# m7a/bo-lz4-ada

Measured on AMD Instinct MI355X. Metric: decompressed MiB/s + achieved HBM GB/s vs roofline, 4MiB-block frame @1/2/4/8 GPU, higher is better.
Workload: dtype u8; 1 GPU; configs[2] size, configs[3] shape: 2048 x 4 MiB independent blocks = 8 GiB decoded, FLG 0x70 (B.Indep|B.Checksum), BD 0x70 (content-checksum variant FLG 0x74: e2e_content_checksum); class=mixed, blocks_total=2048, blocks_per_gpu=2048, block_max=4194304, compressed_bytes_rank0=4214903424, decoded_bytes_rank0=8589934592, parallelism=block-shard x1

## Files before the change

### bo-lz4-ada_amd/csrc/lz4ada_idx.hip

```cpp
#include <hip/hip_runtime.h>
#include <stdint.h>

#include "lz4ada_internal.h"
#include "lz4ada_dev.h"

namespace lz4ada {
namespace idx {

#ifndef LZ4ADA_STORED_NT
#define LZ4ADA_STORED_NT 2
#endif
constexpr int CHUNK = 16384;
constexpr int SUB = 32;
constexpr int BATCH = 64 * SUB;
constexpr int RING = 4 * BATCH;
constexpr int LONG = 256;
constexpr int32_t MAX_RUN = 1 << 28;
#ifndef LZ4ADA_LEAD_SEQ
#define LZ4ADA_LEAD_SEQ 60
#endif
constexpr int32_t LEAD_SEQ = LZ4ADA_LEAD_SEQ;
#ifndef LZ4ADA_LEAD_MAX
#define LZ4ADA_LEAD_MAX 1024
#endif
// ... 844 lines not shown
		has = next_item(S, cp, co, cpart, sub_end, n, o_batch, it);
	if (__any(has)) {
		vm_wait();
		for (;;) {
			const uint64_t m = __ballot(has);
			if (m == 0)
				break;
			const int32_t leader = __builtin_ctzll(m);
			const int32_t ldst = __shfl(it.dst, leader);
			const int32_t llen = __shfl(it.len, leader);
			const int32_t lsrc = __shfl(it.src, leader);
			bool ready;
			if (llen > LONG) {
				if (lsrc >= 0)
					wave_literal(ob, ldst, S, lsrc, llen);
				else
					wave_match(ob, olim, ldst, -lsrc, llen);
				ready = (lane == leader);
			} else {
				ready = has && it.len <= LONG &&
				        (it.src >= 0 || it.dst + it.src + min(-it.src, it.len) <= ldst);
				if (ready) {
					if (it.src >= 0)
						for (int32_t c = 0; c < it.len; c += 16)
							gstore_n(ob + it.dst + c, fetch16(S, it.src + c), min(16, it.len - c));
					else
						lane_match(ob, olim, it.dst, -it.src, it.len);
				}
			}
			vm_wait();
			if (ready)
				has = next_item(S, cp, co, cpart, sub_end, n, o_batch, it);
		}
	}
	return true;
}

constexpr int OW = 4080;
constexpr int ORING = 8192;
constexpr int OMASK = ORING - 1;
constexpr int MAXSEQ = 128;
constexpr int RMAX = MAXSEQ / 64;
constexpr int GC = 1;
constexpr int FLUSH_ST = (OW + 15) / 16 / 64 + 1;
static_assert(2 * OW + 16 <= ORING, "batch + its HBM threshold must fit the ring");
#ifndef LZ4ADA_OW_CUT
#define LZ4ADA_OW_CUT OW
#endif
#ifndef LZ4ADA_SEQ_CUT
#define LZ4ADA_SEQ_CUT MAXSEQ
#endif

struct alignas(16) DecLds {
	uint8_t ring[RING + 16];
	uint8_t oring[ORING];
	uint16_t cst[MAXSEQ];
	uint8_t own[256];
	uint64_t rrec[4 * 64];
	uint64_t ldesc[2 * 64];
	uint32_t plut[16 * 4];
	uint8_t junk[16];
};
static_assert(sizeof(DecLds) <= 20480, "8 waves per CU: at most 20 KiB of LDS per wave");

__device__ __forceinline__ uint8_t* oring_of(DecLds& D) { return D.oring; }
__device__ __forceinline__ const uint8_t* oring_of(const DecLds& D) { return D.oring; }
__device__ __forceinline__ uint8_t* own_of(DecLds& D) { return D.own; }
__device__ __forceinline__ uint64_t* ldesc_of(DecLds& D) { return D.ldesc; }
template <class LD>
struct lds_fast {
	static constexpr bool value = false;
};
template <>
struct lds_fast<DecLds> {
	static constexpr bool value = true;
};
__device__ __forceinline__ uint8_t* junk_of(DecLds& D) { return D.junk; }
__device__ __forceinline__ const uint32_t* plut_of(const DecLds& D) { return D.plut; }
template <class LD>
__device__ __forceinline__ uint8_t* junk_of(LD&) { return nullptr; }
template <class LD>
__device__ __forceinline__ const uint32_t* plut_of(const LD&) { return nullptr; }
template <class LD>
__device__ __forceinline__ constexpr uint32_t omask_of(const LD&) { return OMASK; }

__device__ __forceinline__ void lds_store_bf(uint8_t* p, uint8_t* junk, u32x4 v, uint32_t n)
{
	const uint64_t lo = uint64_t(v.x) | (uint64_t(v.y) << 32);
	const uint64_t hi = uint64_t(v.z) | (uint64_t(v.w) << 32);
	__builtin_memcpy(n >= 16u ? p : junk, &v, 16);
	__builtin_memcpy((n & 8u) ? p : junk, &lo, 8);
	const uint64_t r8 = (n & 8u) ? hi : lo;
	uint8_t* const p4 = p + (n & 8u);
	const uint32_t w4 = uint32_t(r8);
	__builtin_memcpy((n & 4u) ? p4 : junk, &w4, 4);
	const uint32_t r4 = (n & 4u) ? uint32_t(r8 >> 32) : w4;
	uint8_t* const p2 = p4 + (n & 4u);
	const uint16_t w2 = uint16_t(r4);
	__builtin_memcpy((n & 2u) ? p2 : junk, &w2, 2);
	*((n & 1u) ? p2 + (n & 2u) : junk) = uint8_t((n & 2u) ? (r4 >> 16) : r4);
}

template <class LD>
__device__ __forceinline__ void ostore(LD& L, int32_t x, u32x4 v, int32_t n)
{
	const uint32_t a = uint32_t(x) & omask_of(L);
	if constexpr (lds_fast<LD>::value) {
		if (__builtin_expect(!__any(a + uint32_t(n) > omask_of(L) + 1), 1)) {
			lds_store_bf(&oring_of(L)[a], junk_of(L), v, uint32_t(n));
			return;
		}
	}
	if (a + uint32_t(n) <= omask_of(L) + 1) {
		lds_store_n(&oring_of(L)[a], v, n);
		return;
	}
	const uint64_t lo = uint64_t(v.x) | (uint64_t(v.y) << 32);
	const uint64_t hi = uint64_t(v.z) | (uint64_t(v.w) << 32);
	for (int32_t i = 0; i < n; ++i) {
		const uint64_t w = i < 8 ? lo : hi;
		oring_of(L)[(a + uint32_t(i)) & omask_of(L)] = uint8_t(w >> (8 * (i & 7)));
	}
}

template <class LD>
__device__ __forceinline__ u32x4 oload16(const LD& L, int32_t x)
{
	return ring16(oring_of(L), uint32_t(x) & omask_of(L), omask_of(L));
}

constexpr uint64_t pattern_lut()
{
	uint64_t v = 0;
	for (int o = 1; o <= 8; ++o)
		v |= (uint64_t(o * (16 / o)) << (5 * (o - 1))) | (uint64_t(8 % o) << (40 + 2 * (o - 1)));
	return v;
}
constexpr uint64_t PAT_LUT = pattern_lut();

__device__ __forceinline__ void make_pattern16(uint64_t s0, uint64_t s1, int32_t off, u32x4& pv,
                                               int32_t& stp)
{
	uint64_t x, hi;
	if (off <= 8) {
		x = off == 8 ? s0 : (s0 & ((uint64_t(1) << (8 * off)) - 1));
#pragma unroll
		for (int i = 0; i < 3; ++i) {
			const int32_t w = off << i;
			x |= w < 8 ? x << (8 * w) : 0;
		}
		const uint32_t sh = uint32_t(off - 1);
		stp = int32_t((PAT_LUT >> (5 * sh)) & 31u);
		const int32_t r = int32_t((PAT_LUT >> (40 + 2 * sh)) & 3u);
		hi = r == 0 ? x : (x >> (8 * r)) | ((x >> (8 * (8 - off))) << (8 * (8 - r)));
	} else {
		const int32_t r = off - 8;
		x = s0;
		hi = (s1 & ((uint64_t(1) << (8 * r)) - 1)) | (s0 << (8 * r));
		stp = off;
	}
	pv.x = uint32_t(x);
	pv.y = uint32_t(x >> 32);
	pv.z = uint32_t(hi);
	pv.w = uint32_t(hi >> 32);
}

__device__ __forceinline__ u32x4 merge_at(u32x4 a, u32x4 b, int32_t c)
{
	auto m = [c](int32_t d) -> uint32_t {
		const int32_t t = c - 4 * d;
		return t >= 4 ? ~0u : (t <= 0 ? 0u : (1u << (8 * t)) - 1u);
	};
	u32x4 v;
	v.x = (a.x & m(0)) | (b.x & ~m(0));
	v.y = (a.y & m(1)) | (b.y & ~m(1));
	v.z = (a.z & m(2)) | (b.z & ~m(2));
	v.w = (a.w & m(3)) | (b.w & ~m(3));
	return v;
}

__device__ __forceinline__ int32_t pattern_step(int32_t off)
{
	return off <= 8 ? int32_t((PAT_LUT >> (5 * (off - 1))) & 31u) : off;
}

__device__ __forceinline__ void pattern_lut_init(uint32_t* plut)
{
	const uint32_t l = lane_id(), off = l >> 2, d = l & 3u;
	uint32_t sel = 0;
	if (off > 0)
		for (uint32_t t = 0; t < 4; ++t) {
			const uint32_t idx = (4 * d + t) % off;
			uint32_t x = idx;
			if (off > 8 && d == 2 && idx >= 8)
				x = idx - 4;
			if (off >= 12 && d == 3 && idx >= 12)
				x = idx - 8;
			sel |= x << (8 * t);
		}
	plut[l] = sel;
}

__device__ __forceinline__ u32x4 pattern_perm(u32x4 v, int32_t off, const uint32_t* plut)
{
	const u32x4 sel = *reinterpret_cast<const u32x4*>(plut + 4 * off);
	const uint32_t h2 = off <= 8 ? v.y : v.z, h3 = off <= 11 ? v.y : v.w;
	u32x4 o;
	o.x = __builtin_amdgcn_perm(v.y, v.x, sel.x);
	o.y = __builtin_amdgcn_perm(v.y, v.x, sel.y);
	o.z = __builtin_amdgcn_perm(h2, v.x, sel.z);
	o.w = __builtin_amdgcn_perm(h3, v.x, sel.w);
	return o;
}

template <class LD>
__device__ __forceinline__ void ring_match(LD& L, int32_t dst, int32_t off, int32_t len)
{
	const int32_t src = dst - off;
	u32x4 pv = oload16(L, src);
	int32_t stp = 16;
	const bool pat = off < 16 && off < len;
	if (pat) {
		if constexpr (lds_fast<LD>::value) {
			pv = pattern_perm(pv, off, plut_of(L));
			stp = pattern_step(off);
		} else {
			make_pattern16(uint64_t(pv.x) | (uint64_t(pv.y) << 32), uint64_t(pv.z) | (uint64_t(pv.w) << 32),
			               off, pv, stp);
		}
	}
	ostore(L, dst, pv, min(16, len));
	int32_t start = 0;
	for (int32_t x = stp; x < len; x += stp) {
		u32x4 v = pv;
		if (!pat) {
			start += 16;
			if (start >= off)
				start -= off;
			v = oload16(L, src + start);
			if (off - start < 16)
				v = merge_at(v, oload16(L, src + start - off), off - start);
		}
		ostore(L, dst + x, v, min(16, len - x));
	}
}

__device__ __forceinline__ int32_t div_small(int32_t t, int32_t d, int32_t& r)
{
	int32_t q = int32_t(float(t) * __builtin_amdgcn_rcpf(float(d)));
	r = t - q * d;
	if (r < 0) {
		--q;
		r += d;
	}
	if (r >= d) {
		++q;
		r -= d;
	}
	return q;
}


__device__ __forceinline__ int32_t piece_owner(int32_t inc, int32_t t);

template <class LD>
__device__ __forceinline__ int32_t chunk_owner(LD& D, int32_t inc, int32_t np, int32_t t0)
{
	const int32_t lane = int32_t(lane_id());
	const int32_t seed = __popcll(__ballot(inc <= t0));
	uint8_t* own = own_of(D);
	own[lane] = uint8_t(lane == 0 ? seed : 0);
	const int32_t excl = inc - np;
	if (np > 0 && excl >= t0 && excl < t0 + 64)
		own[excl - t0] = uint8_t(lane);
	wave_lds_fence();
	const int32_t v = own[lane];
	wave_lds_fence();
	return wave_incl_max(v);
}

template <class LD>
__device__ __forceinline__ int32_t chunk_owner2(LD& D, int32_t inc0, int32_t np0, int32_t inc1,
                                                int32_t np1, int32_t t0)
{
	const int32_t lane = int32_t(lane_id());
	const int32_t seed = __popcll(__ballot(inc0 <= t0)) + __popcll(__ballot(inc1 <= t0));
	uint8_t* own = own_of(D);
	own[lane] = uint8_t(lane == 0 ? seed : 0);
	const int32_t e0 = inc0 - np0, e1 = inc1 - np1;
	if (np0 > 0 && e0 >= t0 && e0 < t0 + 64)
		own[e0 - t0] = uint8_t(lane);
	if (np1 > 0 && e1 >= t0 && e1 < t0 + 64)
		own[e1 - t0] = uint8_t(64 + lane);
	wave_lds_fence();
	const int32_t v = own[lane];
	wave_lds_fence();
	return wave_incl_max(v);
}

__device__ __forceinline__ int32_t match_pieces(int32_t off, int32_t ml)
{
	if (ml <= 0)
		return 0;
	if (!(off < 16 && off < ml))
		return (ml + 15) >> 4;
	const int32_t stp = pattern_step(off);
	int32_t rr;
	return stp == 16 ? (ml + 15) >> 4 : div_small(ml + stp - 1, stp, rr);
}

#ifndef LZ4ADA_BORROW_SLOTS
#define LZ4ADA_BORROW_SLOTS 2
#endif
constexpr int BORROW_SLOTS = LZ4ADA_BORROW_SLOTS;
static_assert(BORROW_SLOTS >= 0 && BORROW_SLOTS <= 2, "round 0's slots, or both rounds'");

#ifndef LZ4ADA_FWD_ROUNDS
#define LZ4ADA_FWD_ROUNDS 5
#endif
constexpr int FWD_ROUNDS = LZ4ADA_FWD_ROUNDS;
#ifndef LZ4ADA_FWD_PIECES
#define LZ4ADA_FWD_PIECES 0
#endif
constexpr int FWD_PIECES = LZ4ADA_FWD_PIECES;

template <class LD>
__device__ __forceinline__ int32_t ring_pieces(LD& D, const int32_t (&mdst)[RMAX],
                                               const int32_t (&off)[RMAX], const int32_t (&ml)[RMAX],
                                               int32_t o_batch, int32_t glo = INT32_MIN)
{
	int32_t steps = 0;
	const int32_t lane = int32_t(lane_id());
	const int32_t np0 = match_pieces(off[0], ml[0]), np1 = match_pieces(off[1], ml[1]);
	const int32_t inc0 = wave_incl_scan(np0);
	const int32_t tot0 = __shfl(inc0, 63);
	const int32_t inc1 = tot0 + wave_incl_scan(np1);
	const int32_t tot = __shfl(inc1, 63);
	auto pack = [&](int32_t md, int32_t of, int32_t m, int32_t excl) -> uint64_t {
		return uint64_t(uint16_t(md - o_batch)) | (uint64_t(uint16_t(of)) << 16) |
		       (uint64_t(uint16_t(m)) << 32) | (uint64_t(uint16_t(excl)) << 48);
	};
	uint64_t* ldesc = ldesc_of(D);
	ldesc[lane] = pack(mdst[0], off[0], ml[0], inc0 - np0);
	ldesc[64 + lane] = pack(mdst[1], off[1], ml[1], inc1 - np1);
	for (int32_t t0 = 0; t0 < tot; t0 += 64) {
		const int32_t t = t0 + lane;
		const bool act = t < tot;
		const int32_t lo = min(chunk_owner2(D, inc0, np0, inc1, np1, t0), 127);
		const uint64_t dd = ldesc[lo];
		const int32_t od = o_batch + int32_t(dd & 0xffffu);
		const int32_t ooff = int32_t((dd >> 16) & 0xffffu), oml = int32_t((dd >> 32) & 0xffffu);
		const int32_t k = t - int32_t(dd >> 48);
		const bool opat = ooff < 16 && ooff < oml;
		const int32_t ostp = opat ? pattern_step(ooff) : 16;
		const bool wide = !opat && oml > ooff;
		const int32_t pd = od + k * ostp;
		const int32_t pn = min(16, oml - k * ostp);
		const int32_t s_lo = (opat || wide) ? od - ooff : od - ooff + 16 * k;
		const int32_t s_hi = (opat || wide) ? od : s_lo + pn;
		const int32_t pe = act ? pd + pn : INT32_MAX, ps = act ? pd : INT32_MAX;
		int32_t fj1 = 64, fj2 = -1;
		if (!__all(!act || s_hi <= __shfl(ps, 0))) {
			int32_t j1 = 0, c2 = 0;
#pragma unroll
			for (int st = 32; st >= 1; st >>= 1) {
				if (__shfl(pe, j1 + st - 1) <= s_lo)
					j1 += st;
				if (__shfl(ps, c2 + st - 1) < s_hi)
					c2 += st;
			}
			fj1 = j1;
			fj2 = min(c2 - 1, lane - 1);
		}
		int32_t F = 0;
		if (FWD_PIECES > 0 && glo != INT32_MIN) {
			const bool plain = act && !opat && !wide;
			int32_t sh = ooff;
			const int32_t q0 = __shfl(ps, fj1), qe = __shfl(pe, fj1);
			bool fw = act && fj1 == fj2 && q0 <= s_lo && s_hi <= qe && __shfl(int32_t(plain), fj1) != 0;
			for (int r = 0; r < FWD_PIECES && __any(fw); ++r) {
				const int32_t p = fj1;
				const int32_t qs = __shfl(sh, p), q1 = __shfl(fj1, p), q2 = __shfl(fj2, p);
				const bool qf = __shfl(int32_t(fw), p) != 0;
				if (fw && s_lo - F - qs >= glo) {
					F += qs;
					sh = ooff + F;
					fj1 = q1;
					fj2 = q2;
					fw = qf;
				} else {
					fw = false;
				}
			}
		}
		uint64_t dep = 0;
		if (act && fj1 <= fj2)
			dep = (fj2 == 63 ? ~uint64_t(0) : ((uint64_t(2) << fj2) - 1)) & ~((uint64_t(1) << fj1) - 1);
		int32_t rem = 0;
		if (wide)
			div_small(16 * k, ooff, rem);
		const int32_t a1 = (opat ? od - ooff : (wide ? od - ooff + rem : s_lo)) - F;
		const int32_t cut = (wide && ooff - rem < 16) ? ooff - rem : 16;
		bool pend = act;
		for (;;) {
			const uint64_t pm = __ballot(pend);
			if (pm == 0)
				break;
			const bool ready = pend && (dep & pm) == 0;
			if constexpr (lds_fast<LD>::value) {
				u32x4 v = oload16(D, a1);
				if (ready && cut < 16)
					v = merge_at(v, oload16(D, a1 - ooff), cut);
				if (ready && opat)
					v = pattern_perm(v, ooff, plut_of(D));
				ostore(D, pd, v, ready ? pn : 0);
			} else if (ready) {
				u32x4 v = oload16(D, a1);
				if (cut < 16)
					v = merge_at(v, oload16(D, a1 - ooff), cut);
				if (opat) {
					int32_t sstp;
					make_pattern16(uint64_t(v.x) | (uint64_t(v.y) << 32),
					               uint64_t(v.z) | (uint64_t(v.w) << 32), ooff, v, sstp);
				}
				ostore(D, pd, v, pn);
			}
			pend = pend && !ready;
			wave_lds_fence();
			++steps;
		}
	}
	return steps;
}

#ifndef LZ4ADA_RING_LANE_MAX
#define LZ4ADA_RING_LANE_MAX 32
#endif
constexpr int RING_LANE_MAX = LZ4ADA_RING_LANE_MAX;
template <class LD>
__device__ __forceinline__ int32_t ring_lanes(LD& D, int32_t mdst, int32_t off, int32_t ml,
                                           int32_t rbeg, int32_t L, int32_t glo = INT32_MIN)
{
	const int32_t lane = int32_t(lane_id());
	const int32_t src = mdst - off;
	const int32_t dep_end = src + min(off, ml);
	const bool far = ml > 0 && (dep_end <= rbeg || off <= L);
	int32_t steps = 0;
	if (!__any(ml > 0 && !far)) {
		if (far)
			ring_match(D, mdst, off, ml);
		wave_lds_fence();
		return 0;
	}
	bool near = ml > 0;
	const int32_t mend = mdst + ml;
	int32_t j1 = 0, c2 = 0;
#pragma unroll
	for (int st = 32; st >= 1; st >>= 1) {
		if (__shfl(mend, j1 + st - 1) <= src)
			j1 += st;
		if (__shfl(mdst, c2 + st - 1) < dep_end)
			c2 += st;
	}
	int32_t fj1 = far ? 64 : j1, fj2 = far ? -1 : min(c2 - 1, lane - 1);
	int32_t fo = off;
	{
		const int32_t pm = __shfl(mdst, fj1), pe = __shfl(mend, fj1), po = __shfl(off, fj1);
		const bool pn = __shfl(int32_t(near), fj1) != 0;
		bool fw = FWD_ROUNDS > 0 && glo != INT32_MIN && near && off >= ml && fj1 == fj2 && pm <= src &&
		          dep_end <= pe && pn && po >= pe - pm;
		for (int r = 0; r < FWD_ROUNDS && __any(fw); ++r) {
			const int32_t p = fj1;
			const int32_t qo = __shfl(fo, p), q1 = __shfl(fj1, p), q2 = __shfl(fj2, p);
			const bool qf = __shfl(int32_t(fw), p) != 0;
			if (fw && mdst - fo - qo >= glo) {
				fo += qo;
				fj1 = q1;
				fj2 = q2;
				fw = qf;
			} else {
				fw = false;
			}
		}
	}
	uint64_t dep = 0;
	if (near && fj1 <= fj2)
		dep = (fj2 == 63 ? ~uint64_t(0) : ((uint64_t(2) << fj2) - 1)) & ~((uint64_t(1) << fj1) - 1);
	for (;;) {
		const uint64_t pending = __ballot(near);
		if (pending == 0)
			break;
		const bool ready = near && (dep & pending) == 0;
		if (ready) {
			ring_match(D, mdst, fo, ml);
			near = false;
		}
		wave_lds_fence();
		++steps;
	}
	return steps;
}

__device__ __forceinline__ int32_t piece_owner(int32_t inc, int32_t t)
{
	int32_t lo = 0;
#pragma unroll
	for (int st = 32; st >= 1; st >>= 1)
		if (__shfl(inc, lo + st - 1) <= t)
// ... 430 lines not shown
					const int32_t t = t0 + lane;
					const int32_t lo = min(chunk_owner2(D, inc0, nc0, inc1, nc1, t0), 127);
					const uint64_t dd = D.ldesc[lo];
					const int32_t lit = base + int32_t(dd & 0xffffu);
					const int32_t dst = o_batch + int32_t((dd >> 16) & 0xffffu);
					const int32_t L = int32_t((dd >> 32) & 0xffffu);
					const int32_t k = 1 + t - int32_t(dd >> 48);
					const bool has = t < tot;
					ostore(D, dst + 16 * k, ZL ? u32x4{ 0u, 0u, 0u, 0u } : fetch16(S, has ? lit + 16 * k : S.lo),
					       has ? min(16, L - 16 * k) : 0);
				}
			}
		}
		wave_lds_fence();
		ISTAMP(D_LIT);

		int32_t mring[RMAX], oring[RMAX], lring[RMAX];
		__builtin_amdgcn_s_waitcnt(0x0F70);
		ostore(D, rpd, vr, rpn);
#pragma unroll
		for (int r = 0; r < RMAX; ++r) {
			mring[r] = oring[r] = lring[r] = 0;
			if (64 * r < N) {
				const int32_t mdst = rdst[r] + rL[r], off = roff[r], ml = rml[r];
				const bool hbm = ml > 0 && mdst - off < glo;
				static_assert(GC == 1, "one own HBM piece per match");
				ostore(D, hbm ? mdst : o_batch + (bpc[r] & 0xfff), vg[r][0], hbm ? min(16, ml) : bpc[r] >> 12);
				int32_t xoff = off, xml = (ml > 0 && !hbm) ? ml : 0;
				if (d1p) {
					int32_t k1 = 0, sp = S.lo, gq = 0;
					bool fo = false;
					if (ml > 0 && n1 + mdst < off && oph - off < 8) {
						const int32_t dd = oph - off;
						const int32_t ovs = rL[r] > 0 ? 8 * ((rL[r] + 7) >> 3) - rL[r] : rlit[r] & 7;
						if (dd < ovs) {
							k1 = min(ovs - dd, ml);
							if (rL[r] > 0) {
								sp = rlit[r] + rL[r] + dd;
							} else {
								gq = (rlit[r] >> 3) - D1_QBIAS + dd;
								fo = true;
							}
						}
					}
					if (fo && gq >= glo) {
						xoff = mdst - gq;
						xml = k1;
						k1 = 0;
						fo = false;
					}
					u32x4 v = ZL ? u32x4{ 0u, 0u, 0u, 0u } : fetch16(S, sp);
					if (fo)
						__builtin_memcpy(&v, ob + gq, 16);
					ostore(D, mdst, v, k1);
				}
				if (rtot[r] > rfirst[r]) {
					ICOUNT(D_HSLOW_B, r == 0 || rtot[0] <= rfirst[0]);
					ICOUNT(D_HSLOW_P, rtot[r] - rfirst[r]);
					const int32_t nc = hbm ? max(((ml + 15) >> 4) - GC, 0) : 0;
					const int32_t inc = wave_incl_scan(nc);
					for (int32_t t0 = rfirst[r]; t0 < rtot[r]; t0 += 64) {
						const int32_t t = t0 + lane;
						const int32_t lo = piece_owner(inc, t);
						const int32_t k = GC + t - (__shfl(inc, lo) - __shfl(nc, lo));
						const int32_t osrc = __shfl(mdst - off, lo), odst = __shfl(mdst, lo);
						const int32_t oml = __shfl(ml, lo);
						if (t < rtot[r]) {
							u32x4 v;
							__builtin_memcpy(&v, ob + osrc + 16 * k, 16);
							ostore(D, odst + 16 * k, v, min(16, oml - 16 * k));
						}
					}
					__builtin_amdgcn_s_waitcnt(0x0F70);
				}
				mring[r] = mdst;
				oring[r] = xoff;
				lring[r] = xml;
			}
		}
		wave_lds_fence();
		ISTAMP(D_MFAR);
		static_assert(RMAX == 2, "ring dealing pairs two rounds");
		if (__any(lring[0] > RING_LANE_MAX || lring[1] > RING_LANE_MAX)) {
			const int32_t st = ring_pieces(D, mring, oring, lring, o_batch, glo);
			ICOUNT(D_TASKS, 1);
			ICOUNT(D_ROUNDS, st);
#ifdef LZ4ADA_IDX_STAMPS
			{
				const int32_t tot = __shfl(wave_incl_scan(match_pieces(oring[0], lring[0]) +
				                                          match_pieces(oring[1], lring[1])), 63);
				ICOUNT(D_RCHUNKS, (tot + 63) >> 6);
				ICOUNT(D_ROVF_B, tot > 64);
				ICOUNT(D_ROVF_P, max(tot - 64, 0));
			}
#endif
			(void)st;
		} else {
#pragma unroll
			for (int r = 0; r < RMAX; ++r) {
				if (64 * r < N) {
					const int32_t st = ring_lanes(D, mring[r], oring[r], lring[r], rbeg[r], rL[r], glo);
					ICOUNT(D_GBATCHES, 1);
					ICOUNT(D_LANES, st);
					(void)st;
				}
			}
		}
		ISTAMP(D_NEAR);

		{
			const int32_t u0 = o_batch >> 4, u1 = o_end >> 4;
#pragma unroll
			for (int i = 0; i < FLUSH_ST; ++i) {
				const int32_t u = u0 + lane + 64 * i;
				if (u < u1)
					*reinterpret_cast<GLOBAL u32x4*>(ob + (u << 4)) =
					    *reinterpret_cast<const u32x4*>(&D.oring[(u << 4) & OMASK]);
			}
		}
		o_batch = o_end;
		k0 += m;
		ISTAMP(D_FLUSH);
	}
	d1 = __any(d1);
	deep = __any(deep);
	if (ZL)
		hcnt = __shfl(wave_incl_scan(hcnt), 63);
	if (!bad && lane == 0 && (o_batch & 15))
		gstore_n(ob + (o_batch & ~15), *reinterpret_cast<const u32x4*>(&D.oring[(o_batch & ~15) & OMASK]),
		         o_batch & 15);
	if (lane == 0) {
		if (bad) {
			status[b].code = DS_RETRY;
		} else {
			status[b].code = DS_OK;
			status[b].aux = (d1 ? AUX_D1_RISK : 0) | (d1p ? AUX_D1_EMU : 0) | (deep ? AUX_DEEP_HIST : 0);
			status[b].detail = ZL ? hcnt : 0;
			status[b].err_out_pos = 0;
			status[b].out_len = uint32_t(o_batch);
		}
	}
	ISTAMP_FLUSH();
	out_len = bad ? 0 : o_batch;
	return bad ? DS_RETRY : DS_OK;
}

enum KIdxMode : int {
	K_PASS2 = 0,
	K_SERIAL = 1,
	K_HIST = 2,
	K_FUSED = 3,
};

__global__ __launch_bounds__(64) __attribute__((amdgpu_waves_per_eu(2))) void k_decode_idx(const uint8_t* __restrict__ frame,
                                                    uint64_t frame_len,
                                                    const lz4ada_block_desc* __restrict__ desc,
                                                    uint32_t nblocks, uint8_t* __restrict__ tab_all,
                                                    uint8_t* __restrict__ out,
                                                    lz4ada_block_status* __restrict__ status,
                                                    int mode)
{
	__shared__ union {
		DecLds d;
		IdxLds<1> x;
	} U;
	DecLds& D = U.d;
	if (mode == K_FUSED) {
		if (blockIdx.x < nblocks)
			index_block<1>(U.x, frame, frame_len, desc, blockIdx.x, tab_all, status);
		vm_wait();
		__builtin_amdgcn_fence(__ATOMIC_SEQ_CST, "workgroup");
		__syncthreads();
		mode = K_PASS2;
	}
	const bool serial = mode == K_SERIAL;
	int64_t hist = mode == K_HIST ? LINK_HIST : 0;
	uint32_t b = serial ? 0u : blockIdx.x;
	const uint32_t bend = serial ? nblocks : min(blockIdx.x + 1u, nblocks);
	for (; b < bend; ++b) {
		int32_t len;
		const int32_t code = decode_block(D, frame, frame_len, desc, b, tab_all, out, status,
		                                  hist, len);
		if (!serial)
			return;
		vm_wait();
		__syncthreads();
		if (code != DS_OK)
			break;
		if (b + 1 < nblocks && (uint32_t(len) != desc[b].out_cap ||
		                        desc[b + 1].out_off != desc[b].out_off + uint64_t(len))) {
			++b;
			break;
		}
		hist += len;
	}
	if (!serial)
		return;
	for (uint32_t r = b + lane_id(); r < nblocks; r += 64)
		if (status[r].code == DS_OK || r > b)
			status[r].code = DS_RETRY;
}


__global__ __launch_bounds__(64) __attribute__((amdgpu_waves_per_eu(2))) void k_decode_idx_zl(
        const uint8_t* __restrict__ frame, uint64_t frame_len, const lz4ada_block_desc* __restrict__ desc,
        uint32_t nblocks, uint8_t* __restrict__ tab_all, uint8_t* __restrict__ out,
        lz4ada_block_status* __restrict__ status)
{
	__shared__ DecLds D;
	if (blockIdx.x >= nblocks)
		return;
	int32_t len;
	decode_block(D, frame, frame_len, desc, blockIdx.x, tab_all, out, status, LINK_HIST, len, true, true);
}

__global__ __launch_bounds__(64) __attribute__((amdgpu_waves_per_eu(2))) void k_decode_idx_lk(
        const uint8_t* __restrict__ frame, uint64_t frame_len, const lz4ada_block_desc* __restrict__ desc,
        uint32_t nblocks, uint8_t* __restrict__ tab_all, uint8_t* __restrict__ out,
        lz4ada_block_status* __restrict__ status)
{
	__shared__ DecLds D;
	if (blockIdx.x >= nblocks)
		return;
	int32_t len;
	decode_block(D, frame, frame_len, desc, blockIdx.x, tab_all, out, status, LINK_HIST, len, false, true);
}


constexpr int ORING2 = 16384;
constexpr int32_t RFLOOR2 = ORING2 - 2 * OW;
static_assert(OW + 16 + 128 + 16 < RFLOOR2, "the HBM threshold must lie inside the kept window");

struct alignas(16) PpLds2 {
	uint8_t ring[RING + 16];
	uint8_t oring[ORING2];
	uint64_t rrec[4 * 64];
	uint64_t ldesc[2][2 * 64];
	uint16_t cst[2][MAXSEQ];
	uint8_t own[2][256];
	int32_t tok;
	int32_t staged;
	int32_t abort_;
	int32_t pad;
	int32_t done[2];
};

struct WP2 {
	PpLds2& L;
	int32_t w;
};
__device__ __forceinline__ uint8_t* oring_of(WP2& V) { return V.L.oring; }
__device__ __forceinline__ const uint8_t* oring_of(const WP2& V) { return V.L.oring; }
__device__ __forceinline__ uint8_t* own_of(WP2& V) { return V.L.own[V.w]; }
__device__ __forceinline__ uint64_t* ldesc_of(WP2& V) { return V.L.ldesc[V.w]; }
__device__ __forceinline__ constexpr uint32_t omask_of(const WP2&) { return ORING2 - 1; }

__device__ __forceinline__ int32_t lds_peek(const int32_t* p)
{
	return __builtin_amdgcn_readfirstlane(*reinterpret_cast<const volatile int32_t*>(p));
}

__device__ __forceinline__ void lds_publish(int32_t* p, int32_t v)
{
	asm volatile("" ::: "memory");
	__builtin_amdgcn_s_waitcnt(0xC07F);
	*reinterpret_cast<volatile int32_t*>(p) = v;
	asm volatile("" ::: "memory");
}

__device__ __forceinline__ bool lds_wait_ge(int32_t* abort_flag, const int32_t* p, int32_t want)
{
	for (uint32_t it = 0; lds_peek(p) < want; ++it) {
		if (lds_peek(abort_flag))
			return false;
		if (it >= (1u << 24)) {
			lds_publish(abort_flag, 1);
			return false;
		}
		__builtin_amdgcn_s_sleep(1);
	}
	asm volatile("" ::: "memory");
	return true;
}

struct PpCut {
	int32_t m, bytes;
	bool over;
};
__device__ __forceinline__ PpCut pp_cut(const PpLds2& L, int32_t k0, int32_t nsub)
{
	const int32_t k = k0 + int32_t(lane_id());
	const uint64_t rec = k < nsub ? L.rrec[k & 255] : 0;
	const int32_t cnt = int32_t(min(uint32_t(rec >> 32), 1u << 24));
	const int32_t incl = wave_incl_scan(cnt);
	const int32_t incl_s = wave_incl_scan(__popc(uint32_t(rec)));
	PpCut c;
	c.m = __popcll(__ballot(incl <= OW && incl_s <= MAXSEQ));
	c.over = c.m == 0;
	c.m = c.over ? 64 : c.m;
	c.bytes = __shfl(incl, c.m - 1);
	return c;
}

__device__ __forceinline__ void pp_load_chunk(uintptr_t abase, int32_t c, uintptr_t lim, const uint64_t* tab,
                                              int32_t nsub, u32x4& v0, u32x4& v1, uint64_t& r)
{
	load_chunk2(abase, c, lim, v0, v1);
	const int32_t k = 64 * c + int32_t(lane_id());
	r = k < nsub ? __builtin_nontemporal_load(tab + k) : 0;
}

__device__ __forceinline__ void pp_stage_chunk(PpLds2& L, int32_t c, const u32x4& v0, const u32x4& v1,
                                               uint64_t r)
{
	const uint32_t lane = lane_id();
	const uint32_t a = uint32_t(c * BATCH) & (RING - 1);
	*reinterpret_cast<u32x4*>(&L.ring[a + 16 * lane]) = v0;
	*reinterpret_cast<u32x4*>(&L.ring[a + 1024 + 16 * lane]) = v1;
	if (a == 0 && lane == 0)
		*reinterpret_cast<u32x4*>(&L.ring[RING]) = v0;
	L.rrec[64 * (c & 3) + lane] = r;
}

__device__ __forceinline__ int32_t decode_block_pp2(PpLds2& L, const uint8_t* __restrict__ frame,
                                                    uint64_t frame_len,
                                                    const lz4ada_block_desc* __restrict__ desc, uint32_t b,
                                                    const uint8_t* __restrict__ tab_all,
                                                    uint8_t* __restrict__ out)
{
	const int32_t tid = int32_t(threadIdx.x), w = tid >> 6, lane = tid & 63;
	WP2 V{ L, w };
	const lz4ada_block_desc d = desc[b];
	cg8* in = gptr(frame) + d.in_off;
	g8* ob = gptr(out) + d.out_off;
	const int32_t n = int32_t(d.in_len);
	const int32_t cap = int32_t(d.out_cap);
	const uintptr_t lim = reinterpret_cast<uintptr_t>(frame) + frame_len;
	const uintptr_t olim = reinterpret_cast<uintptr_t>(ob) + uintptr_t(cap);
// ... 251 lines not shown
					rpd = od + 16 * k;
					rpn = min(16, oml - 16 * k);
					__builtin_memcpy(&vr, ob + (od - ooff) + 16 * k, 16);
				}
				wave_lds_fence();
			}
		}

		{
#pragma unroll
			for (int r = 0; r < RMAX; ++r)
				if (rL[r] > 0)
					ostore(V, rdst[r], fetch16(S, rlit[r]), min(16, rL[r]));
			const int32_t nc0 = rL[0] > 16 ? (rL[0] - 1) >> 4 : 0;
			const int32_t nc1 = rL[1] > 16 ? (rL[1] - 1) >> 4 : 0;
			if (__any(nc0 > 0 || nc1 > 0)) {
				const int32_t inc0 = wave_incl_scan(nc0);
				const int32_t tot0 = __shfl(inc0, 63);
				const int32_t inc1 = tot0 + wave_incl_scan(nc1);
				const int32_t tot = __shfl(inc1, 63);
				auto pack = [&](int32_t lit, int32_t dst, int32_t Lx, int32_t excl) -> uint64_t {
					return uint64_t(uint16_t(lit - base)) | (uint64_t(uint16_t(dst - ob0)) << 16) |
					       (uint64_t(uint16_t(Lx)) << 32) | (uint64_t(uint16_t(excl)) << 48);
				};
				uint64_t* ldesc = ldesc_of(V);
				ldesc[lane] = pack(rlit[0], rdst[0], rL[0], inc0 - nc0);
				ldesc[64 + lane] = pack(rlit[1], rdst[1], rL[1], inc1 - nc1);
				for (int32_t t0 = 0; t0 < tot; t0 += 64) {
					const int32_t t = t0 + lane;
					const int32_t lo = min(chunk_owner2(V, inc0, nc0, inc1, nc1, t0), 127);
					const uint64_t dd = ldesc[lo];
					const int32_t lit = base + int32_t(dd & 0xffffu);
					const int32_t dst = ob0 + int32_t((dd >> 16) & 0xffffu);
					const int32_t Lx = int32_t((dd >> 32) & 0xffffu);
					const int32_t k = 1 + t - int32_t(dd >> 48);
					if (t < tot)
						ostore(V, dst + 16 * k, fetch16(S, lit + 16 * k), min(16, Lx - 16 * k));
				}
			}
		}
		wave_lds_fence();

		int32_t mring[RMAX], oring[RMAX], lring[RMAX];
		__builtin_amdgcn_s_waitcnt(0x0F70);
		if (rpn > 0)
			ostore(V, rpd, vr, rpn);
#pragma unroll
		for (int r = 0; r < RMAX; ++r) {
			mring[r] = oring[r] = lring[r] = 0;
			if (64 * r < N) {
				const int32_t mdst = rdst[r] + rL[r];
				if (hml[r] > 0)
					ostore(V, mdst, vg[r], min(16, hml[r]));
				if (rtot[r] > rfirst[r]) {
					const int32_t nc = hml[r] > 0 ? max(((hml[r] + 15) >> 4) - 1, 0) : 0;
					const int32_t inc = wave_incl_scan(nc);
					for (int32_t t0 = rfirst[r]; t0 < rtot[r]; t0 += 64) {
						const int32_t t = t0 + lane;
						const int32_t lo = piece_owner(inc, t);
						const int32_t k = 1 + t - (__shfl(inc, lo) - __shfl(nc, lo));
						const int32_t osrc = __shfl(mdst - roff[r], lo), odst = __shfl(mdst, lo);
						const int32_t oml = __shfl(hml[r], lo);
						if (t < rtot[r]) {
							u32x4 v;
							__builtin_memcpy(&v, ob + osrc + 16 * k, 16);
							ostore(V, odst + 16 * k, v, min(16, oml - 16 * k));
						}
					}
					__builtin_amdgcn_s_waitcnt(0x0F70);
				}
				mring[r] = mdst + hml[r];
				oring[r] = roff[r];
				lring[r] = rml[r] - hml[r];
			}
		}
		wave_lds_fence();

		if (!lds_wait_ge(abort_flag, &L.tok, jb - 1)) {
			bad = true;
			break;
		}
		static_assert(RMAX == 2, "ring dealing pairs two rounds");
		if (__any(lring[0] > RING_LANE_MAX || lring[1] > RING_LANE_MAX)) {
			ring_pieces(V, mring, oring, lring, ob0, ob0 - RFLOOR2);
		} else {
#pragma unroll
			for (int r = 0; r < RMAX; ++r)
				if (64 * r < N)
					ring_lanes(V, mring[r], oring[r], lring[r], rbeg[r], rL[r], ob0 - RFLOOR2);
		}
		lds_publish(&L.tok, jb);

		{
			const int32_t u0 = ob0 >> 4, u1 = oe >> 4;
#pragma unroll
			for (int i = 0; i < FLUSH_ST; ++i) {
				const int32_t u = u0 + lane + 64 * i;
				if (u < u1)
					*reinterpret_cast<GLOBAL u32x4*>(ob + (u << 4)) =
					    *reinterpret_cast<const u32x4*>(&L.oring[(u << 4) & WMASK]);
			}
		}
		if (next_over) {
			vm_wait();
			lds_publish(&L.done[w], jb);
		}
	}
	__syncthreads();
	bad = bad || lds_peek(abort_flag) != 0;
	if (!bad && tid == 0 && (o & 15))
		gstore_n(ob + (o & ~15), *reinterpret_cast<const u32x4*>(&L.oring[(o & ~15) & WMASK]), o & 15);
	return bad ? -1 : o;
}

__global__ __launch_bounds__(128) __attribute__((amdgpu_waves_per_eu(2))) void k_decode_pp2(
        const uint8_t* __restrict__ frame, uint64_t frame_len, const lz4ada_block_desc* __restrict__ desc,
        uint32_t nblocks, uint8_t* __restrict__ tab_all, uint8_t* __restrict__ out,
        lz4ada_block_status* __restrict__ status)
{
	__shared__ union {
		PpLds2 d;
		IdxLds<2> x;
	} U;
	if (blockIdx.x >= nblocks)
		return;
	const uint32_t b = blockIdx.x;
	const int32_t tid = int32_t(threadIdx.x), w = tid >> 6;
	index_block<2>(U.x, frame, frame_len, desc, b, tab_all, status);
	vm_wait();
	__builtin_amdgcn_fence(__ATOMIC_SEQ_CST, "workgroup");
	__syncthreads();
	const lz4ada_block_desc d = desc[b];
	if (status[b].code != DS_OK)
		return;
	if (d.flags & LZ4ADA_BLOCK_STORED) {
		const int32_t n = int32_t(d.in_len);
		int32_t c = DS_OK;
		if (n > int32_t(d.out_cap)) {
			c = DS_OUT_OVERFLOW;
		} else {
			Src S0;
			S0.in = gptr(frame) + d.in_off;
			S0.lim = reinterpret_cast<uintptr_t>(frame) + frame_len;
			const int32_t mid = (n >> 1) & ~1023;
			const int32_t c0 = w == 0 ? 0 : mid, c1 = w == 0 ? mid : n;
			if (d.flags & LZ4ADA_BLOCK_HAS_CKSUM)
				wave_literal<0>(gptr(out) + d.out_off, c0, S0, c0, c1 - c0);
			else
				wave_literal<LZ4ADA_STORED_NT>(gptr(out) + d.out_off, c0, S0, c0, c1 - c0);
		}
		if (tid == 0)
			put_status(status[b], c, n);
		return;
	}
	PpLds2& L = U.d;
	if (tid == 0) {
		L.tok = -1;
		L.staged = 0;
		L.abort_ = 0;
		L.done[0] = L.done[1] = -1;
	}
	__syncthreads();
	const int32_t len = decode_block_pp2(L, frame, frame_len, desc, b, tab_all, out);
	if (tid == 0) {
		if (len < 0)
			status[b].code = DS_RETRY;
		else
// ... 125 lines not shown
```

Measured before the change: 635,900 MiB/s.

## Process two match pieces per lane in ring_pieces and drop forwarding path

```diff
diff --git a/bo-lz4-ada_amd/csrc/lz4ada_idx.hip b/bo-lz4-ada_amd/csrc/lz4ada_idx.hip
--- a/bo-lz4-ada_amd/csrc/lz4ada_idx.hip
+++ b/bo-lz4-ada_amd/csrc/lz4ada_idx.hip
@@ -950,7 +950,9 @@
 template <class LD>
 __device__ __forceinline__ const uint32_t* plut_of(const LD&) { return nullptr; }
 template <class LD>
-__device__ __forceinline__ constexpr uint32_t omask_of(const LD&) { return OMASK; }
+constexpr uint32_t omask_v = OMASK;
+template <class LD>
+__device__ __forceinline__ constexpr uint32_t omask_of(const LD&) { return omask_v<LD>; }
 
 __device__ __forceinline__ void lds_store_bf(uint8_t* p, uint8_t* junk, u32x4 v, uint32_t n)
 {
@@ -985,6 +987,7 @@
 	}
 	const uint64_t lo = uint64_t(v.x) | (uint64_t(v.y) << 32);
 	const uint64_t hi = uint64_t(v.z) | (uint64_t(v.w) << 32);
+#pragma clang loop vectorize(disable) unroll(disable)
 	for (int32_t i = 0; i < n; ++i) {
 		const uint64_t w = i < 8 ? lo : hi;
 		oring_of(L)[(a + uint32_t(i)) & omask_of(L)] = uint8_t(w >> (8 * (i & 7)));
@@ -1148,22 +1151,28 @@
 }
 
 template <class LD>
-__device__ __forceinline__ int32_t chunk_owner2(LD& D, int32_t inc0, int32_t np0, int32_t inc1,
-                                                int32_t np1, int32_t t0)
+__device__ __forceinline__ int32_t chunk_owner_marks(LD& D, int32_t seed, int32_t e0, bool nz0, int32_t e1,
+                                                     bool nz1, int32_t t0)
 {
 	const int32_t lane = int32_t(lane_id());
-	const int32_t seed = __popcll(__ballot(inc0 <= t0)) + __popcll(__ballot(inc1 <= t0));
 	uint8_t* own = own_of(D);
 	own[lane] = uint8_t(lane == 0 ? seed : 0);
-	const int32_t e0 = inc0 - np0, e1 = inc1 - np1;
-	if (np0 > 0 && e0 >= t0 && e0 < t0 + 64)
+	if (nz0 && e0 >= t0 && e0 < t0 + 64)
 		own[e0 - t0] = uint8_t(lane);
-	if (np1 > 0 && e1 >= t0 && e1 < t0 + 64)
+	if (nz1 && e1 >= t0 && e1 < t0 + 64)
 		own[e1 - t0] = uint8_t(64 + lane);
 	wave_lds_fence();
 	const int32_t v = own[lane];
 	wave_lds_fence();
 	return wave_incl_max(v);
+}
+
+template <class LD>
+__device__ __forceinline__ int32_t chunk_owner2(LD& D, int32_t inc0, int32_t np0, int32_t inc1,
+                                                int32_t np1, int32_t t0)
+{
+	const int32_t seed = __popcll(__ballot(inc0 <= t0)) + __popcll(__ballot(inc1 <= t0));
+	return chunk_owner_marks(D, seed, inc0 - np0, np0 > 0, inc1 - np1, np1 > 0, t0);
 }
 
 __device__ __forceinline__ int32_t match_pieces(int32_t off, int32_t ml)
@@ -1187,46 +1196,68 @@
 #define LZ4ADA_FWD_ROUNDS 5
 #endif
 constexpr int FWD_ROUNDS = LZ4ADA_FWD_ROUNDS;
-#ifndef LZ4ADA_FWD_PIECES
-#define LZ4ADA_FWD_PIECES 0
-#endif
-constexpr int FWD_PIECES = LZ4ADA_FWD_PIECES;
+
+__device__ __forceinline__ int32_t ring_piece_count(int32_t off, int32_t ml)
+{
+	return (match_pieces(off, ml) + 1) >> 1;
+}
+
+template <class LD>
+__device__ __forceinline__ int32_t chunk_owner_e(LD& D, uint32_t ee, bool nz0, bool nz1, int32_t t0)
+{
+	const int32_t e0 = int32_t(ee & 0xffffu), e1 = int32_t(ee >> 16);
+	const int32_t seed = __popcll(__ballot(e0 <= t0)) + __popcll(__ballot(e1 <= t0)) - 1;
+	return chunk_owner_marks(D, seed, e0, nz0, e1, nz1, t0);
+}
+
+__device__ __forceinline__ void step_state(uint32_t& a, uint32_t& b) { asm volatile("" : "+v"(a), "+v"(b)); }
 
 template <class LD>
 __device__ __forceinline__ int32_t ring_pieces(LD& D, const int32_t (&mdst)[RMAX],
                                                const int32_t (&off)[RMAX], const int32_t (&ml)[RMAX],
-                                               int32_t o_batch, int32_t glo = INT32_MIN)
+                                               int32_t o_batch)
 {
 	int32_t steps = 0;
 	const int32_t lane = int32_t(lane_id());
-	const int32_t np0 = match_pieces(off[0], ml[0]), np1 = match_pieces(off[1], ml[1]);
-	const int32_t inc0 = wave_incl_scan(np0);
-	const int32_t tot0 = __shfl(inc0, 63);
-	const int32_t inc1 = tot0 + wave_incl_scan(np1);
-	const int32_t tot = __shfl(inc1, 63);
-	auto pack = [&](int32_t md, int32_t of, int32_t m, int32_t excl) -> uint64_t {
-		return uint64_t(uint16_t(md - o_batch)) | (uint64_t(uint16_t(of)) << 16) |
-		       (uint64_t(uint16_t(m)) << 32) | (uint64_t(uint16_t(excl)) << 48);
-	};
-	uint64_t* ldesc = ldesc_of(D);
-	ldesc[lane] = pack(mdst[0], off[0], ml[0], inc0 - np0);
-	ldesc[64 + lane] = pack(mdst[1], off[1], ml[1], inc1 - np1);
+	const bool nz0 = ml[0] > 0, nz1 = ml[1] > 0;
+	int32_t tot;
+	uint32_t ee;
+	{
+		const int32_t np0 = ring_piece_count(off[0], ml[0]), np1 = ring_piece_count(off[1], ml[1]);
+		const int32_t inc0 = wave_incl_scan(np0);
+		const int32_t tot0 = __shfl(inc0, 63);
+		const int32_t inc1 = tot0 + wave_incl_scan(np1);
+		tot = __shfl(inc1, 63);
+		auto pack = [&](int32_t md, int32_t of, int32_t m, int32_t excl) -> uint64_t {
+			return uint64_t(uint16_t(md - o_batch)) | (uint64_t(uint16_t(of)) << 16) |
+			       (uint64_t(uint16_t(m)) << 32) | (uint64_t(uint16_t(excl)) << 48);
+		};
+		uint64_t* ldesc = ldesc_of(D);
+		ldesc[lane] = pack(mdst[0], off[0], ml[0], inc0 - np0);
+		ldesc[64 + lane] = pack(mdst[1], off[1], ml[1], inc1 - np1);
+		ee = uint32_t(inc0 - np0) | (uint32_t(inc1 - np1) << 16);
+	}
 	for (int32_t t0 = 0; t0 < tot; t0 += 64) {
 		const int32_t t = t0 + lane;
 		const bool act = t < tot;
-		const int32_t lo = min(chunk_owner2(D, inc0, np0, inc1, np1, t0), 127);
-		const uint64_t dd = ldesc[lo];
+		const int32_t lo = min(chunk_owner_e(D, ee, nz0, nz1, t0), 127);
+		const uint64_t dd = ldesc_of(D)[lo];
 		const int32_t od = o_batch + int32_t(dd & 0xffffu);
 		const int32_t ooff = int32_t((dd >> 16) & 0xffffu), oml = int32_t((dd >> 32) & 0xffffu);
 		const int32_t k = t - int32_t(dd >> 48);
 		const bool opat = ooff < 16 && ooff < oml;
 		const int32_t ostp = opat ? pattern_step(ooff) : 16;
 		const bool wide = !opat && oml > ooff;
-		const int32_t pd = od + k * ostp;
-		const int32_t pn = min(16, oml - k * ostp);
-		const int32_t s_lo = (opat || wide) ? od - ooff : od - ooff + 16 * k;
-		const int32_t s_hi = (opat || wide) ? od : s_lo + pn;
-		const int32_t pe = act ? pd + pn : INT32_MAX, ps = act ? pd : INT32_MAX;
+		const int32_t base = 2 * k * ostp;
+		const int32_t pd = od + base;
+		const int32_t left = oml - base;
+		const bool two = left > 16;
+		const int32_t pd2 = two ? pd + ostp : pd;
+		const int32_t n2 = two ? min(16, left - ostp) : left;
+		const int32_t pe_ = pd2 + n2;
+		const int32_t s_lo = (opat || wide) ? od - ooff : od - ooff + base;
+		const int32_t s_hi = (opat || wide) ? od : s_lo + (pe_ - pd);
+		const int32_t pe = act ? pe_ : INT32_MAX, ps = act ? pd : INT32_MAX;
 		int32_t fj1 = 64, fj2 = -1;
 		if (!__all(!act || s_hi <= __shfl(ps, 0))) {
 			int32_t j1 = 0, c2 = 0;
@@ -1240,58 +1271,72 @@
 			fj1 = j1;
 			fj2 = min(c2 - 1, lane - 1);
 		}
-		int32_t F = 0;
-		if (FWD_PIECES > 0 && glo != INT32_MIN) {
-			const bool plain = act && !opat && !wide;
-			int32_t sh = ooff;
-			const int32_t q0 = __shfl(ps, fj1), qe = __shfl(pe, fj1);
-			bool fw = act && fj1 == fj2 && q0 <= s_lo && s_hi <= qe && __shfl(int32_t(plain), fj1) != 0;
-			for (int r = 0; r < FWD_PIECES && __any(fw); ++r) {
-				const int32_t p = fj1;
-				const int32_t qs = __shfl(sh, p), q1 = __shfl(fj1, p), q2 = __shfl(fj2, p);
-				const bool qf = __shfl(int32_t(fw), p) != 0;
-				if (fw && s_lo - F - qs >= glo) {
-					F += qs;
-					sh = ooff + F;
-					fj1 = q1;
-					fj2 = q2;
-					fw = qf;
-				} else {
-					fw = false;
-				}
-			}
-		}
 		uint64_t dep = 0;
 		if (act && fj1 <= fj2)
 			dep = (fj2 == 63 ? ~uint64_t(0) : ((uint64_t(2) << fj2) - 1)) & ~((uint64_t(1) << fj1) - 1);
-		int32_t rem = 0;
-		if (wide)
-			div_small(16 * k, ooff, rem);
-		const int32_t a1 = (opat ? od - ooff : (wide ? od - ooff + rem : s_lo)) - F;
-		const int32_t cut = (wide && ooff - rem < 16) ? ooff - rem : 16;
+		static_assert(omask_v<LD> < (1u << 14), "ring addresses pack into 14 bits");
+		uint32_t sa, sb;
+		{
+			int32_t rem = 0;
+			if (wide)
+				div_small(base, ooff, rem);
+			const int32_t a1 = opat ? od - ooff : (wide ? od - ooff + rem : s_lo);
+			const int32_t cut1 = (wide && ooff - rem < 16) ? ooff - rem : 16;
+			const bool wrap2 = wide && rem + 16 >= ooff;
+			const int32_t rem2 = rem + 16 - (wrap2 ? ooff : 0);
+			const int32_t cut2 = (wide && ooff - rem2 < 16) ? ooff - rem2 : 16;
+			sa = (uint32_t(a1) & omask_of(D)) | ((uint32_t(pd) & omask_of(D)) << 14) | (uint32_t(ostp - 1) << 28);
+			sb = uint32_t(ooff) | (uint32_t(cut1) << 16) | (uint32_t(cut2) << 21) | (uint32_t(max(n2, 0)) << 26) |
+			     (uint32_t(wrap2) << 31);
+		}
+		const bool ld2 = two && !opat;
 		bool pend = act;
 		for (;;) {
 			const uint64_t pm = __ballot(pend);
 			if (pm == 0)
 				break;
 			const bool ready = pend && (dep & pm) == 0;
+			step_state(sa, sb);
+			const int32_t xa1 = int32_t(sa & 0x3fffu), xpd = int32_t((sa >> 14) & 0x3fffu);
+			const int32_t xoff = int32_t(sb & 0xffffu), xcut1 = int32_t((sb >> 16) & 31u);
+			const int32_t xcut2 = int32_t((sb >> 21) & 31u), xn2 = int32_t((sb >> 26) & 31u);
+			const int32_t xa2 = xa1 + 16 - (int32_t(sb) < 0 ? xoff : 0);
+			const int32_t xpd2 = two ? xpd + int32_t(sa >> 28) + 1 : xpd;
 			if constexpr (lds_fast<LD>::value) {
-				u32x4 v = oload16(D, a1);
-				if (ready && cut < 16)
-					v = merge_at(v, oload16(D, a1 - ooff), cut);
+				u32x4 v = oload16(D, xa1);
+				if (ready && xcut1 < 16)
+					v = merge_at(v, oload16(D, xa1 - xoff), xcut1);
 				if (ready && opat)
-					v = pattern_perm(v, ooff, plut_of(D));
-				ostore(D, pd, v, ready ? pn : 0);
+					v = pattern_perm(v, xoff, plut_of(D));
+				if (__builtin_expect(!__any(ready && two && uint32_t(xpd) + 16u > omask_of(D) + 1), 1))
+					__builtin_memcpy((ready && two) ? &oring_of(D)[xpd] : junk_of(D), &v, 16);
+				else
+					ostore(D, xpd, v, (ready && two) ? 16 : 0);
+				if (__any(ready && ld2)) {
+					u32x4 w = oload16(D, xa2);
+					if (ready && ld2 && xcut2 < 16)
+						w = merge_at(w, oload16(D, xa2 - xoff), xcut2);
+					if (ld2)
+						v = w;
+				}
+				ostore(D, xpd2, v, ready ? xn2 : 0);
 			} else if (ready) {
-				u32x4 v = oload16(D, a1);
-				if (cut < 16)
-					v = merge_at(v, oload16(D, a1 - ooff), cut);
+				u32x4 v = oload16(D, xa1);
+				if (xcut1 < 16)
+					v = merge_at(v, oload16(D, xa1 - xoff), xcut1);
 				if (opat) {
 					int32_t sstp;
 					make_pattern16(uint64_t(v.x) | (uint64_t(v.y) << 32),
-					               uint64_t(v.z) | (uint64_t(v.w) << 32), ooff, v, sstp);
+					               uint64_t(v.z) | (uint64_t(v.w) << 32), xoff, v, sstp);
 				}
-				ostore(D, pd, v, pn);
+				if (two)
+					ostore(D, xpd, v, 16);
+				if (ld2) {
+					v = oload16(D, xa2);
+					if (xcut2 < 16)
+						v = merge_at(v, oload16(D, xa2 - xoff), xcut2);
+				}
+				ostore(D, xpd2, v, xn2);
 			}
 			pend = pend && !ready;
 			wave_lds_fence();
@@ -1888,13 +1933,13 @@
 		ISTAMP(D_MFAR);
 		static_assert(RMAX == 2, "ring dealing pairs two rounds");
 		if (__any(lring[0] > RING_LANE_MAX || lring[1] > RING_LANE_MAX)) {
-			const int32_t st = ring_pieces(D, mring, oring, lring, o_batch, glo);
+			const int32_t st = ring_pieces(D, mring, oring, lring, o_batch);
 			ICOUNT(D_TASKS, 1);
 			ICOUNT(D_ROUNDS, st);
 #ifdef LZ4ADA_IDX_STAMPS
 			{
-				const int32_t tot = __shfl(wave_incl_scan(match_pieces(oring[0], lring[0]) +
-				                                          match_pieces(oring[1], lring[1])), 63);
+				const int32_t tot = __shfl(wave_incl_scan(ring_piece_count(oring[0], lring[0]) +
+				                                          ring_piece_count(oring[1], lring[1])), 63);
 				ICOUNT(D_RCHUNKS, (tot + 63) >> 6);
 				ICOUNT(D_ROVF_B, tot > 64);
 				ICOUNT(D_ROVF_P, max(tot - 64, 0));
@@ -2059,7 +2104,8 @@
 __device__ __forceinline__ const uint8_t* oring_of(const WP2& V) { return V.L.oring; }
 __device__ __forceinline__ uint8_t* own_of(WP2& V) { return V.L.own[V.w]; }
 __device__ __forceinline__ uint64_t* ldesc_of(WP2& V) { return V.L.ldesc[V.w]; }
-__device__ __forceinline__ constexpr uint32_t omask_of(const WP2&) { return ORING2 - 1; }
+template <>
+constexpr uint32_t omask_v<WP2> = ORING2 - 1;
 
 __device__ __forceinline__ int32_t lds_peek(const int32_t* p)
 {
@@ -2477,7 +2523,7 @@
 		}
 		static_assert(RMAX == 2, "ring dealing pairs two rounds");
 		if (__any(lring[0] > RING_LANE_MAX || lring[1] > RING_LANE_MAX)) {
-			ring_pieces(V, mring, oring, lring, ob0, ob0 - RFLOOR2);
+			ring_pieces(V, mring, oring, lring, ob0);
 		} else {
 #pragma unroll
 			for (int r = 0; r < RMAX; ++r)
```

Result: faster. 643,700 MiB/s (median of 6 runs) (+1.2%).
